# Aedelon/MASt3R-SLAM

Measured on AMD Instinct MI355X. Metric: keyframe-pairs/sec (512x512 two-view infer+match+GN), higher is better.
Workload: dtype fp16

## Files before the change

### include/m3slam_model.h

```cpp
#ifndef M3SLAM_MODEL_H
#define M3SLAM_MODEL_H

#include <stdint.h>

#ifdef __cplusplus
extern "C" {
#endif

enum { M3_DT_BF16 = 0, M3_DT_F16 = 1, M3_DT_F16_PVBF16 = 2 };

enum {
    M3_EPI_BF16 = 0,
    M3_EPI_BF16_GELU = 1,
    M3_EPI_F32 = 2,
    M3_EPI_F32_ACCUM = 3,
    M3_EPI_BF16_RELU = 4,
    M3_EPI_BF16_ADD = 5,
    M3_EPI_BF16_ROPE = 6,
    M3_EPI_INPUT_RELU = 0x100
};

typedef struct m3_gemm_desc {
    const void *A, *W, *W1;
    const float *bias, *bias1;
// ... 29 lines not shown
                             int dtype, void *stream);

int m3_dpt_tail_grouped2_dt(const void *X, const void *Wc0, const void *Wc1, const float *bias0, const float *bias1,
                            const void *W40, const void *W41, const float *b40, const float *b41, float *pts,
                            float *conf, const void *zero16, int B, int H, int Wd, int upsample, int dtype,
                            void *stream);

int m3_conv3x3_up_direct_grouped2_dt(const void *X, const void *W0, const void *W1, const float *bias0,
                                     const float *bias1, void *Y, const void *zero16, int B, int H, int Wd, int Cin,
                                     int upsample, int dtype, void *stream);

int m3_conv3x3_direct_grouped2_dt(const void *X, const void *W0, const void *W1, const float *bias0, const float *bias1,
                                  void *Y, const void *R, const void *zero16, int B, int H, int Wd, int Cin, int Cout,
                                  int epilogue, int dtype, void *stream);

int m3_attention_dt(const void *Q, const void *K, const void *V, void *O, int q_row_stride,
                    int kv_row_stride, int o_row_stride, int64_t q_batch_stride,
                    int64_t kv_batch_stride, int64_t o_batch_stride, int nbatch, int heads,
                    int Tq, int Tk, int kv_batch_shift, float scale, int dtype, void *stream);

int m3_attention_prescaled_dt(const void *Q, const void *K, const void *V, void *O, int q_row_stride,
                              int kv_row_stride, int o_row_stride, int64_t q_batch_stride,
                              int64_t kv_batch_stride, int64_t o_batch_stride, int nbatch, int heads,
                              int Tq, int Tk, int kv_batch_shift, int dtype, void *stream);

int m3_rope2d_dt(void *X, const int32_t *pos_yx, const float *cos_sin, int row_stride, int tokens,
                 int heads, int tokens_per_image, int dtype, void *stream);

int m3_layernorm_dt(const float *x, const float *gamma, const float *beta, void *y, int M, int C,
                    float eps, int dtype, void *stream);
// ... 32 lines not shown
```

### mast3r-slam_amd/csrc/conv_tail.hip

```cpp
#include "gemm_common.h"

using namespace m3gemm;

namespace {

constexpr int kThreads = 512;
constexpr int TH = 16, TW = 32;
constexpr int HH = TH + 2, HW = TW + 2;
constexpr int kHaloPix = HH * HW;
constexpr int kHaloBytes = kHaloPix * 128;
constexpr int kWStage = 128 * 128;
constexpr int PH = 11, PW = 19;
constexpr int kPatchBytes = (PH * PW * 128 + 1023) / 1024 * 1024;
constexpr int kLdsBytes = kHaloBytes + 2 * kWStage + kPatchBytes;

struct TailArgs {
    const bf16_t *X;
    const bf16_t *Wc;
    const float *bias;
    const bf16_t *W4;
    const float *b4;
    float *pts, *conf;
    bf16_t *Y;
    const bf16_t *R;
    int cout, relu_in;
    const bf16_t *zero16;
    int B, H, W, IH, IW;
    const bf16_t *Wc2, *W42;
    const float *bias2, *b42;
};

enum { EP_PLAIN = 0 , EP_TAIL = 1 , EP_RELU = 2 ,
       EP_ADD = 3  };

template <int DT, bool UPS, int CIN, int EP>
__global__ void __launch_bounds__(kThreads, 2)
k_conv_tail(const TailArgs ain) {
    constexpr bool TAIL = EP == EP_TAIL;
    static_assert(CIN % 64 == 0 && (TAIL ? CIN == 128 : true), "64-channel steps; the fused tail is the 128-channel head.2");
    constexpr int NQ = CIN / 64;
    TailArgs a = ain;
    if (blockIdx.y == 1) {
        a.Wc = ain.Wc2; a.W4 = ain.W42; a.bias = ain.bias2; a.b4 = ain.b42;
        a.X = ain.X + (size_t)ain.B * ain.IH * ain.IW * CIN;
        if (TAIL) {
            a.pts = ain.pts + (size_t)ain.B * ain.H * ain.W * 3;
            a.conf = ain.conf + (size_t)ain.B * ain.H * ain.W;
        } else {
            a.Y = ain.Y + (size_t)ain.B * ain.H * ain.W * ain.cout;
            if (EP == EP_ADD) a.R = ain.R + (size_t)ain.B * ain.H * ain.W * ain.cout;
        }
    }
    if (!TAIL) {
        const int z = blockIdx.z;
        a.Wc += (size_t)z * 128 * 9 * CIN;
        if (a.bias) a.bias += z * 128;
        a.Y += z * 128;
        if (EP == EP_ADD) a.R += z * 128;
    }
    extern __shared__ __attribute__((aligned(16))) unsigned char lds[];
    unsigned char *halo = lds, *wst = lds + kHaloBytes, *patch = lds + kHaloBytes + 2 * kWStage;
    const int tid = threadIdx.x, lane = tid & 63, wave = tid >> 6;
    const int wp = wave >> 1, wc = wave & 1;
    const int tiles_x = (a.W + TW - 1) / TW, tiles_y = a.H / TH;
    const int nwg = tiles_x * tiles_y * a.B;
    const int bid = xcd_remap(blockIdx.x, nwg);
    const int b = bid / (tiles_x * tiles_y), trem = bid - b * tiles_x * tiles_y;
    const int ty = trem / tiles_x, tx = trem - ty * tiles_x;
    const int oy0 = ty * TH, ox0 = tx * TW;
    const bf16_t *img = a.X + (size_t)b * a.IH * a.IW * CIN;

    auto stage_w = [&](int tap, int half, int buf) {
        unsigned char *base = wst + buf * kWStage;
#pragma unroll
        for (int i = 0; i < 2; ++i) {
            const int slot = i * kThreads + tid;
            const int row = slot >> 3, cp = slot & 7;
            const int c = half * 8 + (cp ^ ((row >> 1) & 7));
            glds16(a.Wc + ((size_t)row * 9 + tap) * CIN + c * 8, base + i * (kThreads * 16) + wave * 1024);
// ... 47 lines not shown
                q11.q = *reinterpret_cast<const uint4 *>(p + ((y1 - py0) * PW + (x1 - px0)) * 128);
#pragma unroll
                for (int k = 0; k < 4; ++k) {
                    const float tl = lo16<DT>(q00.w[k]) * (1.f - wx) + lo16<DT>(q01.w[k]) * wx;
                    const float bl = lo16<DT>(q10.w[k]) * (1.f - wx) + lo16<DT>(q11.w[k]) * wx;
                    const float th = hi16<DT>(q00.w[k]) * (1.f - wx) + hi16<DT>(q01.w[k]) * wx;
                    const float bh = hi16<DT>(q10.w[k]) * (1.f - wx) + hi16<DT>(q11.w[k]) * wx;
                    r.w[k] = pack16<DT>(tl * (1.f - wy) + bl * wy, th * (1.f - wy) + bh * wy);
                }
                o = r.q;
            }
            *reinterpret_cast<uint4 *>(halo + (size_t)slot * 16) = o;
        }
    };

    f32x4 acc[8][4];
#pragma unroll
    for (int i = 0; i < 8; ++i)
#pragma unroll
        for (int j = 0; j < 4; ++j) acc[i][j] = f32x4{0.f, 0.f, 0.f, 0.f};
    const int frow = lane & 15, fch = lane >> 4;
    int w_off[4];
#pragma unroll
    for (int j = 0; j < 4; ++j) {
        const int r = wc * 64 + j * 16 + frow;
        w_off[j] = r * 128 + ((fch ^ ((r >> 1) & 7)) << 4);
    }

    const int group = wave >> 2;
    bf16x8 af[8], wf[4];
    const int pix_of_row = (int)((0x3D9F2A40E6C851B7ULL >> (4 * frow)) & 15);
    auto col_offset = [&](int hx) { return hx * 128 + ((fch ^ ((hx >> 1) & 7)) << 4); };
    auto read_frags = [&](int g, int tap, int ks) {
        const int ky = tap / 3, kx = tap - ky * 3;
        const unsigned char *wsrc = wst + (g & 1) * kWStage;
        const int flip = ks << 6;
        const int c0 = col_offset(pix_of_row + kx) ^ flip;
        const int c1 = col_offset(16 + pix_of_row + kx) ^ flip;
        const unsigned char *rowp = halo + (wp * 4 + ky) * (HW * 128);
#pragma unroll
        for (int j = 0; j < 4; ++j) wf[j] = *reinterpret_cast<const bf16x8 *>(wsrc + (w_off[j] ^ flip));
#pragma unroll
        for (int i = 0; i < 8; ++i)
            af[i] = *reinterpret_cast<const bf16x8 *>(rowp + (i >> 1) * (HW * 128) + ((i & 1) ? c1 : c0));
        if (!TAIL && a.relu_in) {
#pragma unroll
            for (int i = 0; i < 8; ++i) af[i] = relu_frag(af[i]);
        }
    };
    auto mfma_all = [&]() {
        __builtin_amdgcn_s_setprio(1);
#pragma unroll
        for (int i = 0; i < 8; ++i)
#pragma unroll
            for (int j = 0; j < 4; ++j) acc[i][j] = mfma16<DT>(wf[j], af[i], acc[i][j]);
        __builtin_amdgcn_s_setprio(0);
    };
    auto phase_end = [&]() {
        __builtin_amdgcn_sched_barrier(0);
        __builtin_amdgcn_s_barrier();
        __builtin_amdgcn_sched_barrier(0);
    };
    auto phase_end_wait = [&]() {
        __builtin_amdgcn_sched_barrier(0);
        asm volatile("s_waitcnt vmcnt(0)" ::: "memory");
        __builtin_amdgcn_s_barrier();
        __builtin_amdgcn_sched_barrier(0);
    };
    auto prefetch_w = [&](int g) { if (g + 1 < 9 * NQ) stage_w((g + 1) % 9, (g + 1) / 9, (g + 1) & 1); };
    auto run_half = [&](int half) {
        if (group == 0) {
#pragma unroll 1
            for (int tap = 0; tap < 9; ++tap) {
                const int g = half * 9 + tap;
                read_frags(g, tap, 0);
                prefetch_w(g);
                asm volatile("s_waitcnt lgkmcnt(0)" ::: "memory");
                phase_end();
                mfma_all();
                phase_end();
                read_frags(g, tap, 1);
                asm volatile("s_waitcnt lgkmcnt(0)" ::: "memory");
                phase_end();
                mfma_all();
                phase_end_wait();
            }
            phase_end();
        } else {
#pragma unroll 1
            for (int tap = 0; tap < 9; ++tap) {
                const int g = half * 9 + tap;
                if (tap > 0) mfma_all();
                phase_end();
                read_frags(g, tap, 0);
                prefetch_w(g);
                asm volatile("s_waitcnt lgkmcnt(0)" ::: "memory");
                phase_end();
                mfma_all();
                phase_end();
                read_frags(g, tap, 1);
                asm volatile("s_waitcnt lgkmcnt(0)" ::: "memory");
                phase_end_wait();
            }
            mfma_all();
            phase_end();
        }
    };

    stage_w(0, 0, 0);
    if (UPS) stage_patch(0); else stage_halo_direct(0);
    asm volatile("s_waitcnt vmcnt(0)" ::: "memory");
    lds_barrier();
#pragma unroll 1
    for (int q = 0; q < NQ; ++q) {
        if (UPS) {
            blend_halo();
            lds_barrier();
            if (q + 1 < NQ) stage_patch(q + 1);
        } else if (q > 0) {
            stage_halo_direct(q);
            asm volatile("s_waitcnt vmcnt(0)" ::: "memory");
            lds_barrier();
        }
        run_half(q);
    }

    if constexpr (EP == EP_ADD) {
        const int r = lane & 15, gq = lane >> 4;
        constexpr int RS = 272;
        unsigned char *wl = halo + wave * (32 * RS);
        float4 bj[4];
#pragma unroll
        for (int j = 0; j < 4; ++j)
            bj[j] = a.bias ? *reinterpret_cast<const float4 *>(a.bias + wc * 64 + j * 16 + gq * 4) : make_float4(0.f, 0.f, 0.f, 0.f);
        auto pix = [&](int pass, int rl, int &oy, int &ox) {
            const int i = pass * 2 + (rl >> 4);
            oy = oy0 + wp * 4 + (i >> 1);
            ox = ox0 + (i & 1) * 16 + (int)((0x3D9F2A40E6C851B7ULL >> (4 * (rl & 15))) & 15);
        };
        uint4 q[2][4];
        auto load_resid = [&](int pass, uint4 (&dst)[4]) {
#pragma unroll
            for (int it = 0; it < 4; ++it) {
                const int c = it * 64 + lane, rl = c >> 3, ch = c & 7;
                int oy, ox;
                pix(pass, rl, oy, ox);
                ox = ox < a.W ? ox : a.W - 1;
                dst[it] = *reinterpret_cast<const uint4 *>(a.R + (((size_t)b * a.H + oy) * a.W + ox) * a.cout + wc * 64 + ch * 8);
            }
        };
        load_resid(0, q[0]);
#pragma unroll
        for (int pass = 0; pass < 4; ++pass) {
            if (pass + 1 < 4) load_resid(pass + 1, q[(pass + 1) & 1]);
#pragma unroll
            for (int ii = 0; ii < 2; ++ii)
#pragma unroll
                for (int j = 0; j < 4; ++j) {
                    const f32x4 v = acc[pass * 2 + ii][j];
                    *reinterpret_cast<float4 *>(wl + (ii * 16 + r) * RS + ((j * 4 + gq) << 4)) =
                        make_float4(v[0] + bj[j].x, v[1] + bj[j].y, v[2] + bj[j].z, v[3] + bj[j].w);
                }
            asm volatile("s_waitcnt lgkmcnt(0)" ::: "memory");
#pragma unroll
            for (int it = 0; it < 4; ++it) {
                const int c = it * 64 + lane, rl = c >> 3, ch = c & 7;
                const float4 f0 = *reinterpret_cast<const float4 *>(wl + rl * RS + ch * 32);
                const float4 f1 = *reinterpret_cast<const float4 *>(wl + rl * RS + ch * 32 + 16);
                const uint4 u = q[pass & 1][it];
                uint4 o;
                o.x = pack16<DT>(f0.x + lo16<DT>(u.x), f0.y + hi16<DT>(u.x));
                o.y = pack16<DT>(f0.z + lo16<DT>(u.y), f0.w + hi16<DT>(u.y));
                o.z = pack16<DT>(f1.x + lo16<DT>(u.z), f1.y + hi16<DT>(u.z));
                o.w = pack16<DT>(f1.z + lo16<DT>(u.w), f1.w + hi16<DT>(u.w));
                int oy, ox;
                pix(pass, rl, oy, ox);
                if (ox < a.W)
                    *reinterpret_cast<uint4 *>(a.Y + (((size_t)b * a.H + oy) * a.W + ox) * a.cout + wc * 64 + ch * 8) = o;
            }
            asm volatile("" ::: "memory");
        }
    } else if constexpr (!TAIL) {
        const int r = lane & 15, gq = lane >> 4;
        unsigned char *wl = halo + wave * 8192;
        float4 bj[4];
#pragma unroll
        for (int j = 0; j < 4; ++j)
            bj[j] = a.bias ? *reinterpret_cast<const float4 *>(a.bias + wc * 64 + j * 16 + gq * 4) : make_float4(0.f, 0.f, 0.f, 0.f);
#pragma unroll
        for (int pass = 0; pass < 2; ++pass) {
#pragma unroll
            for (int ii = 0; ii < 4; ++ii)
#pragma unroll
                for (int j = 0; j < 4; ++j) {
                    f32x4 v = acc[pass * 4 + ii][j];
                    v[0] += bj[j].x; v[1] += bj[j].y; v[2] += bj[j].z; v[3] += bj[j].w;
                    if (EP == EP_RELU) {
#pragma unroll
                        for (int e = 0; e < 4; ++e) v[e] = v[e] > 0.f ? v[e] : 0.f;
                    }
                    uint2 pk;
                    pk.x = pack16<DT>(v[0], v[1]); pk.y = pack16<DT>(v[2], v[3]);
                    *reinterpret_cast<uint2 *>(wl + (ii * 16 + r) * 128 + (((j * 2 + (gq >> 1)) ^ ((r >> 1) & 7)) << 4) + (((gq ^ r) & 1) << 3)) = pk;
                }
            asm volatile("s_waitcnt lgkmcnt(0)" ::: "memory");
#pragma unroll
            for (int it = 0; it < 8; ++it) {
                const int c = it * 64 + lane, rl = c >> 3, ch = c & 7;
                uint4 v = *reinterpret_cast<const uint4 *>(wl + rl * 128 + ((ch ^ ((rl >> 1) & 7)) << 4));
                if (rl & 1) v = uint4{v.z, v.w, v.x, v.y};
                const int i = pass * 4 + (rl >> 4);
                const int oy = oy0 + wp * 4 + (i >> 1);
                const int ox = ox0 + (i & 1) * 16 + (int)((0x3D9F2A40E6C851B7ULL >> (4 * (rl & 15))) & 15);
                if (ox < a.W)
                    *reinterpret_cast<uint4 *>(a.Y + (((size_t)b * a.H + oy) * a.W + ox) * a.cout + wc * 64 + ch * 8) = v;
            }
            asm volatile("" ::: "memory");
        }
    } else {
        const int r = lane & 15, gq = lane >> 4;
        float part[8][4];
    #pragma unroll
        for (int i = 0; i < 8; ++i)
    #pragma unroll
            for (int o = 0; o < 4; ++o) part[i][o] = 0.f;
    #pragma unroll
        for (int j = 0; j < 4; ++j) {
            const int n = wc * 64 + j * 16 + gq * 4;
            const float4 bq = a.bias ? *reinterpret_cast<const float4 *>(a.bias + n) : make_float4(0.f, 0.f, 0.f, 0.f);
// ... 36 lines not shown
            if (ox < a.W) {
                const float x = p0.x + p1.x + a.b4[0], y = p0.y + p1.y + a.b4[1];
                const float z = p0.z + p1.z + a.b4[2], c = p0.w + p1.w + a.b4[3];
                const float d = sqrtf(x * x + y * y + z * z);
                const float sc = expm1f(d) / fmaxf(d, 1e-8f);
                const size_t m = ((size_t)b * a.H + oy) * a.W + ox;
                a.pts[3 * m + 0] = x * sc; a.pts[3 * m + 1] = y * sc; a.pts[3 * m + 2] = z * sc;
                a.conf[m] = 1.0f + expf(c);
            }
        }
    }
}

}

extern "C" {

static int dpt_tail_launch(const void *X, const void *Wc, const float *bias, const void *W4, const float *b4,
                           const void *Wc2, const float *bias2, const void *W42, const float *b42, float *pts,
                           float *conf, void *Y, const void *R, const void *zero16, int B, int H, int W, int cin, int cout,
                           int ep, int relu_in, int upsample, int dtype, void *stream) {
    const int groups = Wc2 ? 2 : 1;
    const bool tail = ep == EP_TAIL;
    M3_REQUIRE(X && Wc && zero16 && B > 0 && H > 0 && W > 0 && H % 16 == 0 && W % 16 == 0);
    M3_REQUIRE(tail ? (W4 && b4 && pts && conf && cin == 128 && !Y)
                    : (Y && (cin == 128 || cin == 256) && (cout == 128 || cout == 256) && (ep == EP_PLAIN || ep == EP_RELU || ep == EP_ADD)));
    M3_REQUIRE((ep == EP_ADD) == (R != nullptr) && (!upsample || ep == EP_PLAIN || tail));
    M3_REQUIRE(groups == 1 || ((!tail || (W42 && b42)) && (bias == nullptr) == (bias2 == nullptr)));
    M3_REQUIRE((dtype == DT_BF16 || dtype == DT_F16) && (!upsample || (H % 2 == 0 && W % 2 == 0)));
    M3_REQUIRE((int64_t)groups * B * H * W < (1ll << 31));
    M3_REQUIRE(reinterpret_cast<uintptr_t>(X) % 16 == 0 && reinterpret_cast<uintptr_t>(Wc) % 16 == 0 &&
               reinterpret_cast<uintptr_t>(Y) % 16 == 0 && reinterpret_cast<uintptr_t>(R) % 16 == 0);
    TailArgs a;
    a.Wc2 = (const bf16_t *)Wc2; a.W42 = (const bf16_t *)W42; a.bias2 = bias2; a.b42 = b42;
    a.X = (const bf16_t *)X; a.Wc = (const bf16_t *)Wc; a.bias = bias; a.W4 = (const bf16_t *)W4; a.b4 = b4;
    a.pts = pts; a.conf = conf; a.Y = (bf16_t *)Y; a.R = (const bf16_t *)R; a.cout = tail ? 128 : cout; a.relu_in = relu_in;
    a.zero16 = (const bf16_t *)zero16; a.B = B; a.H = H; a.W = W;
    a.IH = upsample ? H / 2 : H; a.IW = upsample ? W / 2 : W;
    const dim3 grid((unsigned)((H / TH) * ((W + TW - 1) / TW) * B), groups, tail ? 1 : cout / 128), blk(kThreads);
    hipStream_t st = (hipStream_t)stream;
#define M3_TAIL(DTV, UP, CI, EPV)                                                                                \
    do {                                                                                                         \
        static M3AttrOnce once;                                                                                  \
        int dev__;                                                                                               \
        if (m3_attr_need(once, &dev__)) {                                                                        \
            M3_CHECK_HIP(hipFuncSetAttribute(reinterpret_cast<const void *>(&k_conv_tail<DTV, UP, CI, EPV>),     \
                                             hipFuncAttributeMaxDynamicSharedMemorySize, kLdsBytes), "m3_dpt_tail/attr"); \
            m3_attr_done(once, dev__);                                                                           \
        }                                                                                                        \
        hipLaunchKernelGGL((k_conv_tail<DTV, UP, CI, EPV>), grid, blk, kLdsBytes, st, a);                        \
    } while (0)
#define M3_TAIL_DT(UP, CI, EPV) do { if (dtype == DT_F16) M3_TAIL(DT_F16, UP, CI, EPV); else M3_TAIL(DT_BF16, UP, CI, EPV); } while (0)
    if (tail) { if (upsample) M3_TAIL_DT(true, 128, EP_TAIL); else M3_TAIL_DT(false, 128, EP_TAIL); }
    else if (ep == EP_PLAIN && cin == 128) { if (upsample) M3_TAIL_DT(true, 128, EP_PLAIN); else M3_TAIL_DT(false, 128, EP_PLAIN); }
    else if (ep == EP_PLAIN) { if (upsample) M3_TAIL_DT(true, 256, EP_PLAIN); else M3_TAIL_DT(false, 256, EP_PLAIN); }
    else if (ep == EP_RELU) { if (cin == 128) M3_TAIL_DT(false, 128, EP_RELU); else M3_TAIL_DT(false, 256, EP_RELU); }
    else { if (cin == 128) M3_TAIL_DT(false, 128, EP_ADD); else M3_TAIL_DT(false, 256, EP_ADD); }
#undef M3_TAIL_DT
#undef M3_TAIL
    M3_CHECK_LAUNCH("m3_dpt_tail");
    return M3_OK;
}

int m3_dpt_tail_grouped2_dt(const void *X, const void *Wc0, const void *Wc1, const float *bias0, const float *bias1,
                            const void *W40, const void *W41, const float *b40, const float *b41, float *pts,
                            float *conf, const void *zero16, int B, int H, int W, int upsample, int dtype, void *stream) {
    M3_REQUIRE(pts && conf && (Wc1 == nullptr) == (W41 == nullptr));
    if (!Wc1) bias1 = b41 = nullptr;
    return dpt_tail_launch(X, Wc0, bias0, W40, b40, Wc1, bias1, W41, b41, pts, conf, nullptr, nullptr, zero16, B, H, W, 128, 128,
                           EP_TAIL, 0, upsample, dtype, stream);
}

int m3_conv3x3_up_direct_grouped2_dt(const void *X, const void *Wc0, const void *Wc1, const float *bias0, const float *bias1,
                                     void *Y, const void *zero16, int B, int H, int W, int Cin, int upsample, int dtype,
                                     void *stream) {
    M3_REQUIRE(Y != nullptr);
    return dpt_tail_launch(X, Wc0, bias0, nullptr, nullptr, Wc1, Wc1 ? bias1 : nullptr, nullptr, nullptr, nullptr, nullptr, Y,
                           nullptr, zero16, B, H, W, Cin, 128, EP_PLAIN, 0, upsample, dtype, stream);
}

int m3_conv3x3_direct_grouped2_dt(const void *X, const void *W0, const void *W1, const float *bias0, const float *bias1,
                                  void *Y, const void *R, const void *zero16, int B, int H, int W, int Cin, int Cout,
                                  int epilogue, int dtype, void *stream) {
    const int relu_in = (epilogue & 0x100) ? 1 : 0;
    const int e = epilogue & 0xff;
    M3_REQUIRE(Y != nullptr && (e == M3_EPI_BF16 || e == M3_EPI_BF16_RELU || e == M3_EPI_BF16_ADD));
    const int ep = e == M3_EPI_BF16 ? EP_PLAIN : (e == M3_EPI_BF16_RELU ? EP_RELU : EP_ADD);
    return dpt_tail_launch(X, W0, bias0, nullptr, nullptr, W1, bias1, nullptr, nullptr, nullptr, nullptr, Y, R, zero16, B, H, W,
                           Cin, Cout, ep, relu_in, 0, dtype, stream);
}

}
```

### mast3r-slam_amd/csrc/gemm.hip

```cpp
#include <atomic>
#include "gemm_common.h"
#include <cmath>
#include <stdlib.h>

using namespace m3gemm;

namespace {

constexpr int BM = 128, BN = 128;
constexpr int kThreads = 256;

#ifndef M3_GEMM64_STAGES
#define M3_GEMM64_STAGES 2
#endif
constexpr int k_gemm_stages(int T) { return T == 64 ? M3_GEMM64_STAGES : 2; }

template <int MODE , int EPI, int T, int DT, bool SLICED = false>
__global__ void __launch_bounds__(kThreads)
k_gemm(const GemmArgs gin) {
    constexpr int BM = T, BN = T;
    constexpr int NT = T / 32;
    constexpr int kStageBytes = (BM + BN) * BK * 2;
    constexpr int STAGES = k_gemm_stages(T);
    static_assert(4 * (NT == 4 ? 9216 : 4608) + BM * 8 + kRopeTableRows * 128 <= STAGES * kStageBytes, "row table + RoPE table behind the scratch");
// ... 446 lines not shown
        a.rope_pmax = (d->rope_max_pos > 0 && d->rope_max_pos <= kRopeTableRows) ? d->rope_max_pos : 0;
    }
    a.C16 = d->c16; a.stats_out = d->stats_out; a.stats_gstride = d->stats_gstride;
    a.R_lo = d->r_lo; a.C_lo = d->c_lo;
    a.ln_stats = d->ln_stats; a.ln_colsum = d->ln_colsum; a.ln_colsum2 = d->ln_colsum1; a.ln_slots = d->ln_slots;
    a.ln_eps = d->ln_eps; a.ln_gstride = d->ln_gstride;
    if (d->ln_stats) {
        const int top = ln_top_width(d->K);
        a.ln_tops = d->K / top;
        a.ln_gsz = d->ln_slots / a.ln_tops;
    }
    a.stats_w = d->stats_out ? ln_store_width(d->M, d->N, groups) : 0;
    return launch_dense(a, epi, (hipStream_t)stream);
}

int64_t m3_conv3x3_splitk_bytes(int B, int H, int Wd, int Cin, int Cout, int stride) {
    if (B <= 0 || H <= 0 || Wd <= 0 || Cin <= 0 || Cout <= 0 || (stride != 1 && stride != 2)) return 0;
    const int OH = (H + 2 - 3) / stride + 1, OW = (Wd + 2 - 3) / stride + 1;
    const int S = pick_splits(OH * OW, Cout, 9 * Cin);
    return S > 1 ? (int64_t)S * B * OH * OW * Cout * 4 : 0;
}

int m3_conv3x3_grouped2_dt(const void *X, const void *W0, const void *W1, const float *bias0, const float *bias1,
                           void *Y, const void *R, const void *zero16, int B, int H, int Wd, int Cin, int Cout,
                           int stride, int epilogue, void *splitk_ws, int64_t splitk_ws_bytes, int dtype, void *stream) {
    const int relu_in = (epilogue & 0x100) ? 1 : 0;
    epilogue &= 0xff;
    M3_REQUIRE(X && W0 && Y && zero16 && B > 0 && H > 0 && Wd > 0 && Cin > 0 && Cout > 0 && dt_ok(dtype));
    M3_REQUIRE(Cin % BK == 0 && Cout % 4 == 0 && (stride == 1 || stride == 2) && epilogue != EPI_BF16_ROPE);
    M3_REQUIRE(!((epilogue == EPI_F32_ACCUM || epilogue == EPI_BF16_ADD) && !R));
// ... 39 lines not shown
```

### mast3r-slam_amd/mast3r_slam/ops.py

```python
from __future__ import annotations

import os

import ctypes as C

import torch
from torch.utils.weak import WeakTensorKeyDictionary

from . import _ffi

EPI_BF16, EPI_BF16_GELU, EPI_F32, EPI_F32_ACCUM, EPI_BF16_RELU, EPI_BF16_ADD, EPI_BF16_ROPE = range(7)
EPI_INPUT_RELU = 0x100
_F32_EPIS = (EPI_F32, EPI_F32_ACCUM)

_zero16 = {}

H16 = (torch.bfloat16, torch.float16)
DT_CODE = {torch.bfloat16: 0, torch.float16: 1}
DT_F16_PVBF16 = 2


def _pv_code(dt: int, pv_bf16: bool) -> int:
    if not pv_bf16:
        return dt
# ... 96 lines not shown

def conv3x3_ex(x, w, bias=None, epi: int = EPI_BF16, stride: int = 1, resid=None, out=None, relu_input: bool = False, direct=None,
             w1=None, bias1=None):
    x = _ffi.check(x, H16, "x")
    lead = _lead(x, w1, "B,H,W,Cin")
    g = len(lead) + 1
    b, h, wd, cin = x.shape[-4:]
    w = _ffi.check(w, H16, "w", (None, 3, 3, cin))
    cout = w.shape[0]
    w1 = _opt(w1, H16, "w1", tuple(w.shape))
    dt = _same16(x, w, w1)
    oh, ow = (h + 2 - 3) // stride + 1, (wd + 2 - 3) // stride + 1
    odt = torch.float32 if epi in _F32_EPIS else x.dtype
    bias, bias1 = _opt(bias, torch.float32, "bias", (cout,)), _opt(bias1, torch.float32, "bias1", (cout,))
    resid = _opt(resid, odt, "resid", lead + (b, oh, ow, cout))
    if out is None and direct is not False and epi in (EPI_BF16, EPI_BF16_RELU, EPI_BF16_ADD) and (direct or conv3x3_direct_ok(x, cout, stride)):
        return _conv3x3_direct(x, w, w1, bias, bias1, epi, resid, relu_input)
    if out is None:
        out = torch.empty(lead + (b, oh, ow, cout), dtype=odt, device=x.device)
    ws_bytes = g * int(_ffi.lib().m3_conv3x3_splitk_bytes(b, h, wd, cin, cout, stride))
    ws = torch.empty(ws_bytes, dtype=torch.uint8, device=x.device) if ws_bytes > 0 else None
    e0 = _prof_begin()
    _ffi.call("m3_conv3x3_grouped2_dt", _ffi.ptr(x), _ffi.ptr(w), _ffi.ptr(w1), _ffi.ptr(bias), _ffi.ptr(bias1), _ffi.ptr(out),
              _ffi.ptr(resid), _ffi.ptr(zero_page(x.device)), b, h, wd, cin, cout, stride,
              epi | (EPI_INPUT_RELU if relu_input else 0), _ffi.ptr(ws), ws_bytes, dt, _ffi.stream_ptr())
    _prof_end(e0, "conv3x3", 2.0 * g * b * oh * ow * cout * 9 * cin,
              g * (2.0 * (b * h * wd * cin + cout * 9 * cin) + out.element_size() * b * oh * ow * cout * (1 if resid is None else 2)),
              f"conv3x3{' x2' if g == 2 else ''} {b}x{h}x{wd} {cin}->{cout} s{stride} epi{epi} splitk_ws={ws_bytes}")
    return out


def _conv3x3_direct(x, w0, w1, b0, b1, epi, resid, relu_input):
    grouped = x.dim() == 5
    b, h, wd, cin = x.shape[-4:]
    cout = w0.shape[0]
    dt = _same16(x, w0, w1)
    out = torch.empty(tuple(x.shape[:-1]) + (cout,), dtype=x.dtype, device=x.device)
    e0 = _prof_begin()
    _ffi.call("m3_conv3x3_direct_grouped2_dt", _ffi.ptr(x), _ffi.ptr(w0), _ffi.ptr(w1), _ffi.ptr(b0), _ffi.ptr(b1), _ffi.ptr(out),
              _ffi.ptr(resid), _ffi.ptr(zero_page(x.device)), b, h, wd, cin, cout, epi | (EPI_INPUT_RELU if relu_input else 0), dt,
              _ffi.stream_ptr())
    g = 2 if grouped else 1
    _prof_end(e0, "conv_direct", 2.0 * g * b * h * wd * cout * 9 * cin,
              g * (2.0 * (b * h * wd * cin + cout * 9 * cin) + 2.0 * b * h * wd * cout * (1 if resid is None else 2)),
              f"conv3x3 direct{' x2' if grouped else ''} {b}x{h}x{wd} {cin}->{cout} epi{epi}")
    return out


def conv3x3(x: torch.Tensor, w: torch.Tensor, bias=None, epi: int = EPI_BF16, stride: int = 1, resid=None, out=None,
            relu_input: bool = False, direct=None):
    return conv3x3_ex(x, w, bias, epi, stride, resid, out, relu_input, direct)


def conv3x3_grouped2(x, w0, w1, b0, b1, epi: int = EPI_BF16, stride: int = 1, resid=None, relu_input: bool = False, direct=None):
    return conv3x3_ex(x, w0, b0, epi, stride, resid, None, relu_input, direct, w1=_ffi.check(w1, H16, "w1"), bias1=b1)


def conv3x3_relu_head4(x: torch.Tensor, w: torch.Tensor, bias, w4: torch.Tensor, b4: torch.Tensor):
    x = _ffi.check(x, H16, "x")
    b, h, wd, cin = x.shape
# ... 16 lines not shown
DIRECT_CONV_MIN_WGS = None


def _direct_conv_min_wgs() -> int:
    return int(DIRECT_CONV_MIN_WGS) if DIRECT_CONV_MIN_WGS is not None else int(_ffi.lib().m3_device_cu_count())


def conv3x3_direct_ok(x, cout: int, stride: int = 1) -> bool:
    g = 2 if x.dim() == 5 else 1
    b, h, w, cin = x.shape[-4:]
    if stride != 1 or cin not in (128, 256) or cout not in (128, 256) or h % 16 or w % 16 or os.environ.get("M3_DIRECT_CONV", "1") == "0":
        return False
    if int(_ffi.lib().m3_conv3x3_splitk_bytes(1, h, w, cin, cout, 1)) > 0:
        return False
    return (h // 16) * ((w + 31) // 32) * b * (cout // 128) * g >= _direct_conv_min_wgs()


def conv3x3_up_direct_ex(x, w, bias, upsample: bool = True, w1=None, bias1=None):
    x = _ffi.check(x, H16, "x")
    lead = _lead(x, w1, "B,h,w,Cin")
    g = len(lead) + 1
    b, ih, iw, cin = x.shape[-4:]
    w, w1 = _ffi.check(w, H16, "w", (128, 3, 3, cin)), _opt(w1, H16, "w1", (128, 3, 3, cin))
    dt = _same16(x, w, w1)
    bias, bias1 = _opt(bias, torch.float32, "bias", (128,)), _opt(bias1, torch.float32, "bias1", (128,))
    h, wd = (2 * ih, 2 * iw) if upsample else (ih, iw)
    out = torch.empty(lead + (b, h, wd, 128), dtype=x.dtype, device=x.device)
    e0 = _prof_begin()
    _ffi.call("m3_conv3x3_up_direct_grouped2_dt", _ffi.ptr(x), _ffi.ptr(w), _ffi.ptr(w1), _ffi.ptr(bias), _ffi.ptr(bias1), _ffi.ptr(out),
              _ffi.ptr(zero_page(x.device)), b, h, wd, cin, 1 if upsample else 0, dt, _ffi.stream_ptr())
# ... 362 lines not shown
```

Measured before the change: 294.8.

## Add 4-row direct conv tiles with sliced accumulation for small-spatial convs

Adds a 4-row tile variant of the direct 3x3 conv kernel that handles convs which previously fell back to split-K GEMM (Cin 192/384/768, and small spatial sizes). The accumulation is split into slices that are summed in registers to match the split-K summation order. A new routing function picks the tile size from the CU count and the split-K heuristic. It also adds a 16-row path for Cin=192. This avoids the split-K workspace and reduction passes, at the cost of more register pressure and lower per-workgroup reuse.

Result: no change. 295.8 (median of 6 runs) (+0.3%).

```diff
diff --git a/include/m3slam_model.h b/include/m3slam_model.h
--- a/include/m3slam_model.h
+++ b/include/m3slam_model.h
@@ -67,6 +67,14 @@
                                   void *Y, const void *R, const void *zero16, int B, int H, int Wd, int Cin, int Cout,
                                   int epilogue, int dtype, void *stream);
 
+int m3_conv3x3_direct_tile_grouped2_dt(const void *X, const void *W0, const void *W1, const float *bias0, const float *bias1,
+                                       void *Y, const void *R, const void *zero16, int B, int H, int Wd, int Cin, int Cout,
+                                       int epilogue, int tile, int dtype, void *stream);
+
+int m3_conv3x3_small_route(int groups, int B, int H, int Wd, int Cin, int Cout, int stride, int epilogue);
+
+int m3_conv3x3_splits(int pix_per_image, int Cout, int K);
+
 int m3_attention_dt(const void *Q, const void *K, const void *V, void *O, int q_row_stride,
                     int kv_row_stride, int o_row_stride, int64_t q_batch_stride,
                     int64_t kv_batch_stride, int64_t o_batch_stride, int nbatch, int heads,
diff --git a/mast3r-slam_amd/csrc/conv_tail.hip b/mast3r-slam_amd/csrc/conv_tail.hip
--- a/mast3r-slam_amd/csrc/conv_tail.hip
+++ b/mast3r-slam_amd/csrc/conv_tail.hip
@@ -5,14 +5,16 @@
 namespace {
 
 constexpr int kThreads = 512;
-constexpr int TH = 16, TW = 32;
-constexpr int HH = TH + 2, HW = TW + 2;
-constexpr int kHaloPix = HH * HW;
-constexpr int kHaloBytes = kHaloPix * 128;
+constexpr int TW = 32, HW = TW + 2;
+constexpr int halo_bytes(int th) { return (th + 2) * HW * 128; }
 constexpr int kWStage = 128 * 128;
 constexpr int PH = 11, PW = 19;
 constexpr int kPatchBytes = (PH * PW * 128 + 1023) / 1024 * 1024;
-constexpr int kLdsBytes = kHaloBytes + 2 * kWStage + kPatchBytes;
+constexpr int kEpiAddBytes = 8 * 32 * 272;
+constexpr int lds_bytes(int th, bool ups, bool add = false) {
+    const int k = halo_bytes(th) + 2 * kWStage + (ups ? kPatchBytes : 0);
+    return add && k < kEpiAddBytes ? kEpiAddBytes : k;
+}
 
 struct TailArgs {
     const bf16_t *X;
@@ -24,6 +26,7 @@
     bf16_t *Y;
     const bf16_t *R;
     int cout, relu_in;
+    int slices;
     const bf16_t *zero16;
     int B, H, W, IH, IW;
     const bf16_t *Wc2, *W42;
@@ -33,11 +36,16 @@
 enum { EP_PLAIN = 0 , EP_TAIL = 1 , EP_RELU = 2 ,
        EP_ADD = 3  };
 
-template <int DT, bool UPS, int CIN, int EP>
+template <int DT, bool UPS, int CIN, int EP, int TH = 16, bool SLICED = false>
 __global__ void __launch_bounds__(kThreads, 2)
 k_conv_tail(const TailArgs ain) {
     constexpr bool TAIL = EP == EP_TAIL;
     static_assert(CIN % 64 == 0 && (TAIL ? CIN == 128 : true), "64-channel steps; the fused tail is the 128-channel head.2");
+    static_assert((TH == 16 && !SLICED) || (TH == 4 && SLICED && !UPS && !TAIL), "16-row tiles, or 4-row tiles with sliced accumulation");
+    constexpr int HH = TH + 2, kHaloPix = HH * HW, kHaloBytes = halo_bytes(TH);
+    constexpr int RPW = TH / 4;
+    constexpr int NI = 2 * RPW;
+    constexpr int TPP = NI < 4 ? NI : 4;
     constexpr int NQ = CIN / 64;
     TailArgs a = ain;
     if (blockIdx.y == 1) {
@@ -62,7 +70,7 @@
     unsigned char *halo = lds, *wst = lds + kHaloBytes, *patch = lds + kHaloBytes + 2 * kWStage;
     const int tid = threadIdx.x, lane = tid & 63, wave = tid >> 6;
     const int wp = wave >> 1, wc = wave & 1;
-    const int tiles_x = (a.W + TW - 1) / TW, tiles_y = a.H / TH;
+    const int tiles_x = (a.W + TW - 1) / TW, tiles_y = (a.H + TH - 1) / TH;
     const int nwg = tiles_x * tiles_y * a.B;
     const int bid = xcd_remap(blockIdx.x, nwg);
     const int b = bid / (tiles_x * tiles_y), trem = bid - b * tiles_x * tiles_y;
@@ -140,11 +148,28 @@
         }
     };
 
-    f32x4 acc[8][4];
-#pragma unroll
-    for (int i = 0; i < 8; ++i)
+    f32x4 acc[NI][4];
+#pragma unroll
+    for (int i = 0; i < NI; ++i)
 #pragma unroll
         for (int j = 0; j < 4; ++j) acc[i][j] = f32x4{0.f, 0.f, 0.f, 0.f};
+    f32x4 tot[SLICED ? NI : 1][SLICED ? 4 : 1];
+    int slice = 0, slice_end = SLICED ? 9 * NQ * 1 / a.slices : 0;
+    auto fold_slice = [&](int gdone) {
+        if constexpr (SLICED) {
+            if (gdone + 1 == slice_end) {
+#pragma unroll
+                for (int i = 0; i < NI; ++i)
+#pragma unroll
+                    for (int j = 0; j < 4; ++j) {
+                        tot[i][j] = slice == 0 ? acc[i][j] : tot[i][j] + acc[i][j];
+                        acc[i][j] = f32x4{0.f, 0.f, 0.f, 0.f};
+                    }
+                ++slice;
+                slice_end = (int)((long long)(9 * NQ) * (slice + 1) / a.slices);
+            }
+        }
+    };
     const int frow = lane & 15, fch = lane >> 4;
     int w_off[4];
 #pragma unroll
@@ -154,30 +179,31 @@
     }
 
     const int group = wave >> 2;
-    bf16x8 af[8], wf[4];
+    constexpr bool WIDE = TH == 16;
+    bf16x8 af[NI], wf[4], af1[WIDE ? 1 : NI], wf1[WIDE ? 1 : 4];
     const int pix_of_row = (int)((0x3D9F2A40E6C851B7ULL >> (4 * frow)) & 15);
     auto col_offset = [&](int hx) { return hx * 128 + ((fch ^ ((hx >> 1) & 7)) << 4); };
-    auto read_frags = [&](int g, int tap, int ks) {
+    auto read_frags = [&](int g, int tap, int ks, auto &af, auto &wf) {
         const int ky = tap / 3, kx = tap - ky * 3;
         const unsigned char *wsrc = wst + (g & 1) * kWStage;
         const int flip = ks << 6;
         const int c0 = col_offset(pix_of_row + kx) ^ flip;
         const int c1 = col_offset(16 + pix_of_row + kx) ^ flip;
-        const unsigned char *rowp = halo + (wp * 4 + ky) * (HW * 128);
+        const unsigned char *rowp = halo + (wp * RPW + ky) * (HW * 128);
 #pragma unroll
         for (int j = 0; j < 4; ++j) wf[j] = *reinterpret_cast<const bf16x8 *>(wsrc + (w_off[j] ^ flip));
 #pragma unroll
-        for (int i = 0; i < 8; ++i)
+        for (int i = 0; i < NI; ++i)
             af[i] = *reinterpret_cast<const bf16x8 *>(rowp + (i >> 1) * (HW * 128) + ((i & 1) ? c1 : c0));
         if (!TAIL && a.relu_in) {
 #pragma unroll
-            for (int i = 0; i < 8; ++i) af[i] = relu_frag(af[i]);
-        }
-    };
-    auto mfma_all = [&]() {
+            for (int i = 0; i < NI; ++i) af[i] = relu_frag(af[i]);
+        }
+    };
+    auto mfma_all = [&](const auto &af, const auto &wf) {
         __builtin_amdgcn_s_setprio(1);
 #pragma unroll
-        for (int i = 0; i < 8; ++i)
+        for (int i = 0; i < NI; ++i)
 #pragma unroll
             for (int j = 0; j < 4; ++j) acc[i][j] = mfma16<DT>(wf[j], af[i], acc[i][j]);
         __builtin_amdgcn_s_setprio(0);
@@ -194,21 +220,21 @@
         __builtin_amdgcn_sched_barrier(0);
     };
     auto prefetch_w = [&](int g) { if (g + 1 < 9 * NQ) stage_w((g + 1) % 9, (g + 1) / 9, (g + 1) & 1); };
-    auto run_half = [&](int half) {
+    auto run_half_small = [&](int half) {
+        auto read_both = [&](int g, int tap) {
+            read_frags(g, tap, 0, af, wf);
+            read_frags(g, tap, 1, af1, wf1);
+            asm volatile("s_waitcnt lgkmcnt(0)" ::: "memory");
+        };
+        auto mfma_both = [&](int gdone) { mfma_all(af, wf); mfma_all(af1, wf1); fold_slice(gdone); };
         if (group == 0) {
 #pragma unroll 1
             for (int tap = 0; tap < 9; ++tap) {
                 const int g = half * 9 + tap;
-                read_frags(g, tap, 0);
                 prefetch_w(g);
-                asm volatile("s_waitcnt lgkmcnt(0)" ::: "memory");
-                phase_end();
-                mfma_all();
-                phase_end();
-                read_frags(g, tap, 1);
-                asm volatile("s_waitcnt lgkmcnt(0)" ::: "memory");
-                phase_end();
-                mfma_all();
+                read_both(g, tap);
+                phase_end();
+                mfma_both(g);
                 phase_end_wait();
             }
             phase_end();
@@ -216,19 +242,54 @@
 #pragma unroll 1
             for (int tap = 0; tap < 9; ++tap) {
                 const int g = half * 9 + tap;
-                if (tap > 0) mfma_all();
-                phase_end();
-                read_frags(g, tap, 0);
+                prefetch_w(g);
+                if (tap > 0) mfma_both(g - 1);
+                phase_end();
+                read_both(g, tap);
+                phase_end_wait();
+            }
+            mfma_both(half * 9 + 8);
+            phase_end();
+        }
+    };
+    auto run_half = [&](int half) {
+        if constexpr (!WIDE) { run_half_small(half); return; }
+        if (group == 0) {
+#pragma unroll 1
+            for (int tap = 0; tap < 9; ++tap) {
+                const int g = half * 9 + tap;
+                read_frags(g, tap, 0, af, wf);
                 prefetch_w(g);
                 asm volatile("s_waitcnt lgkmcnt(0)" ::: "memory");
                 phase_end();
-                mfma_all();
-                phase_end();
-                read_frags(g, tap, 1);
+                mfma_all(af, wf);
+                phase_end();
+                read_frags(g, tap, 1, af, wf);
+                asm volatile("s_waitcnt lgkmcnt(0)" ::: "memory");
+                phase_end();
+                mfma_all(af, wf);
+                fold_slice(g);
+                phase_end_wait();
+            }
+            phase_end();
+        } else {
+#pragma unroll 1
+            for (int tap = 0; tap < 9; ++tap) {
+                const int g = half * 9 + tap;
+                if (tap > 0) { mfma_all(af, wf); fold_slice(g - 1); }
+                phase_end();
+                read_frags(g, tap, 0, af, wf);
+                prefetch_w(g);
+                asm volatile("s_waitcnt lgkmcnt(0)" ::: "memory");
+                phase_end();
+                mfma_all(af, wf);
+                phase_end();
+                read_frags(g, tap, 1, af, wf);
                 asm volatile("s_waitcnt lgkmcnt(0)" ::: "memory");
                 phase_end_wait();
             }
-            mfma_all();
+            mfma_all(af, wf);
+            fold_slice(half * 9 + 8);
             phase_end();
         }
     };
@@ -250,8 +311,15 @@
         }
         run_half(q);
     }
+    if constexpr (SLICED) {
+#pragma unroll
+        for (int i = 0; i < NI; ++i)
+#pragma unroll
+            for (int j = 0; j < 4; ++j) acc[i][j] = tot[i][j];
+    }
 
     if constexpr (EP == EP_ADD) {
+        static_assert(kEpiAddBytes <= lds_bytes(TH, UPS, true), "epilogue scratch");
         const int r = lane & 15, gq = lane >> 4;
         constexpr int RS = 272;
         unsigned char *wl = halo + wave * (32 * RS);
@@ -261,7 +329,7 @@
             bj[j] = a.bias ? *reinterpret_cast<const float4 *>(a.bias + wc * 64 + j * 16 + gq * 4) : make_float4(0.f, 0.f, 0.f, 0.f);
         auto pix = [&](int pass, int rl, int &oy, int &ox) {
             const int i = pass * 2 + (rl >> 4);
-            oy = oy0 + wp * 4 + (i >> 1);
+            oy = oy0 + wp * RPW + (i >> 1);
             ox = ox0 + (i & 1) * 16 + (int)((0x3D9F2A40E6C851B7ULL >> (4 * (rl & 15))) & 15);
         };
         uint4 q[2][4];
@@ -272,13 +340,14 @@
                 int oy, ox;
                 pix(pass, rl, oy, ox);
                 ox = ox < a.W ? ox : a.W - 1;
+                oy = oy < a.H ? oy : a.H - 1;
                 dst[it] = *reinterpret_cast<const uint4 *>(a.R + (((size_t)b * a.H + oy) * a.W + ox) * a.cout + wc * 64 + ch * 8);
             }
         };
         load_resid(0, q[0]);
 #pragma unroll
-        for (int pass = 0; pass < 4; ++pass) {
-            if (pass + 1 < 4) load_resid(pass + 1, q[(pass + 1) & 1]);
+        for (int pass = 0; pass < NI / 2; ++pass) {
+            if (pass + 1 < NI / 2) load_resid(pass + 1, q[(pass + 1) & 1]);
 #pragma unroll
             for (int ii = 0; ii < 2; ++ii)
 #pragma unroll
@@ -301,25 +370,26 @@
                 o.w = pack16<DT>(f1.z + lo16<DT>(u.w), f1.w + hi16<DT>(u.w));
                 int oy, ox;
                 pix(pass, rl, oy, ox);
-                if (ox < a.W)
+                if (ox < a.W && oy < a.H)
                     *reinterpret_cast<uint4 *>(a.Y + (((size_t)b * a.H + oy) * a.W + ox) * a.cout + wc * 64 + ch * 8) = o;
             }
             asm volatile("" ::: "memory");
         }
     } else if constexpr (!TAIL) {
+        static_assert(8 * TPP * 2048 <= kHaloBytes + 2 * kWStage, "epilogue scratch (4-row tile: over the halo into the dead weight stages)");
         const int r = lane & 15, gq = lane >> 4;
-        unsigned char *wl = halo + wave * 8192;
+        unsigned char *wl = halo + wave * (TPP * 2048);
         float4 bj[4];
 #pragma unroll
         for (int j = 0; j < 4; ++j)
             bj[j] = a.bias ? *reinterpret_cast<const float4 *>(a.bias + wc * 64 + j * 16 + gq * 4) : make_float4(0.f, 0.f, 0.f, 0.f);
 #pragma unroll
-        for (int pass = 0; pass < 2; ++pass) {
-#pragma unroll
-            for (int ii = 0; ii < 4; ++ii)
+        for (int pass = 0; pass < NI / TPP; ++pass) {
+#pragma unroll
+            for (int ii = 0; ii < TPP; ++ii)
 #pragma unroll
                 for (int j = 0; j < 4; ++j) {
-                    f32x4 v = acc[pass * 4 + ii][j];
+                    f32x4 v = acc[pass * TPP + ii][j];
                     v[0] += bj[j].x; v[1] += bj[j].y; v[2] += bj[j].z; v[3] += bj[j].w;
                     if (EP == EP_RELU) {
 #pragma unroll
@@ -331,14 +401,14 @@
                 }
             asm volatile("s_waitcnt lgkmcnt(0)" ::: "memory");
 #pragma unroll
-            for (int it = 0; it < 8; ++it) {
+            for (int it = 0; it < 2 * TPP; ++it) {
                 const int c = it * 64 + lane, rl = c >> 3, ch = c & 7;
                 uint4 v = *reinterpret_cast<const uint4 *>(wl + rl * 128 + ((ch ^ ((rl >> 1) & 7)) << 4));
                 if (rl & 1) v = uint4{v.z, v.w, v.x, v.y};
-                const int i = pass * 4 + (rl >> 4);
-                const int oy = oy0 + wp * 4 + (i >> 1);
+                const int i = pass * TPP + (rl >> 4);
+                const int oy = oy0 + wp * RPW + (i >> 1);
                 const int ox = ox0 + (i & 1) * 16 + (int)((0x3D9F2A40E6C851B7ULL >> (4 * (rl & 15))) & 15);
-                if (ox < a.W)
+                if (ox < a.W && oy < a.H)
                     *reinterpret_cast<uint4 *>(a.Y + (((size_t)b * a.H + oy) * a.W + ox) * a.cout + wc * 64 + ch * 8) = v;
             }
             asm volatile("" ::: "memory");
@@ -405,17 +475,25 @@
 
 }
 
+static bool small_tile_has(int cin, int ep) {
+    return ep == EP_PLAIN ? (cin == 192 || cin == 384 || cin == 768) : ((ep == EP_RELU || ep == EP_ADD) && cin == 256);
+}
+static bool wide_tile_has(int cin, int ep) { return cin == 128 || cin == 256 || (cin == 192 && ep == EP_PLAIN); }
+
 extern "C" {
+
+int m3_conv3x3_splits(int pix_per_image, int Cout, int K);
 
 static int dpt_tail_launch(const void *X, const void *Wc, const float *bias, const void *W4, const float *b4,
                            const void *Wc2, const float *bias2, const void *W42, const float *b42, float *pts,
                            float *conf, void *Y, const void *R, const void *zero16, int B, int H, int W, int cin, int cout,
-                           int ep, int relu_in, int upsample, int dtype, void *stream) {
+                           int ep, int relu_in, int upsample, int dtype, void *stream, int th = 16, int slices = 1) {
     const int groups = Wc2 ? 2 : 1;
     const bool tail = ep == EP_TAIL;
-    M3_REQUIRE(X && Wc && zero16 && B > 0 && H > 0 && W > 0 && H % 16 == 0 && W % 16 == 0);
+    M3_REQUIRE(X && Wc && zero16 && B > 0 && H > 0 && W > 0 && ((H % 16 == 0 && W % 16 == 0) || (!tail && !upsample)));
     M3_REQUIRE(tail ? (W4 && b4 && pts && conf && cin == 128 && !Y)
-                    : (Y && (cin == 128 || cin == 256) && (cout == 128 || cout == 256) && (ep == EP_PLAIN || ep == EP_RELU || ep == EP_ADD)));
+                    : (Y && cout > 0 && cout % 128 == 0 && (ep == EP_PLAIN || ep == EP_RELU || ep == EP_ADD)));
+    M3_REQUIRE(th == 16 ? (wide_tile_has(cin, ep) && slices == 1) : (th == 4 && !tail && !upsample && small_tile_has(cin, ep) && slices >= 1));
     M3_REQUIRE((ep == EP_ADD) == (R != nullptr) && (!upsample || ep == EP_PLAIN || tail));
     M3_REQUIRE(groups == 1 || ((!tail || (W42 && b42)) && (bias == nullptr) == (bias2 == nullptr)));
     M3_REQUIRE((dtype == DT_BF16 || dtype == DT_F16) && (!upsample || (H % 2 == 0 && W % 2 == 0)));
@@ -426,29 +504,47 @@
     a.Wc2 = (const bf16_t *)Wc2; a.W42 = (const bf16_t *)W42; a.bias2 = bias2; a.b42 = b42;
     a.X = (const bf16_t *)X; a.Wc = (const bf16_t *)Wc; a.bias = bias; a.W4 = (const bf16_t *)W4; a.b4 = b4;
     a.pts = pts; a.conf = conf; a.Y = (bf16_t *)Y; a.R = (const bf16_t *)R; a.cout = tail ? 128 : cout; a.relu_in = relu_in;
+    a.slices = slices;
     a.zero16 = (const bf16_t *)zero16; a.B = B; a.H = H; a.W = W;
     a.IH = upsample ? H / 2 : H; a.IW = upsample ? W / 2 : W;
-    const dim3 grid((unsigned)((H / TH) * ((W + TW - 1) / TW) * B), groups, tail ? 1 : cout / 128), blk(kThreads);
+    const int64_t nwg = (int64_t)((H + th - 1) / th) * ((W + TW - 1) / TW) * B;
+    M3_REQUIRE(nwg < (1ll << 31) && cout / 128 <= 65535);
+    const dim3 grid((unsigned)nwg, groups, tail ? 1 : cout / 128), blk(kThreads);
     hipStream_t st = (hipStream_t)stream;
-#define M3_TAIL(DTV, UP, CI, EPV)                                                                                \
+#define M3_TAIL_K(UP, ...)                                                                                       \
     do {                                                                                                         \
         static M3AttrOnce once;                                                                                  \
         int dev__;                                                                                               \
+        constexpr int kLds__ = lds_bytes(th__, UP, add__);                                                            \
         if (m3_attr_need(once, &dev__)) {                                                                        \
-            M3_CHECK_HIP(hipFuncSetAttribute(reinterpret_cast<const void *>(&k_conv_tail<DTV, UP, CI, EPV>),     \
-                                             hipFuncAttributeMaxDynamicSharedMemorySize, kLdsBytes), "m3_dpt_tail/attr"); \
+            M3_CHECK_HIP(hipFuncSetAttribute(reinterpret_cast<const void *>(&k_conv_tail<__VA_ARGS__>),          \
+                                             hipFuncAttributeMaxDynamicSharedMemorySize, kLds__), "m3_dpt_tail/attr"); \
             m3_attr_done(once, dev__);                                                                           \
         }                                                                                                        \
-        hipLaunchKernelGGL((k_conv_tail<DTV, UP, CI, EPV>), grid, blk, kLdsBytes, st, a);                        \
+        hipLaunchKernelGGL((k_conv_tail<__VA_ARGS__>), grid, blk, kLds__, st, a);                                \
     } while (0)
+#define M3_TAIL(DTV, UP, CI, EPV) do { constexpr int th__ = 16; constexpr bool add__ = EPV == EP_ADD; M3_TAIL_K(UP, DTV, UP, CI, EPV); } while (0)
+#define M3_SMALL(DTV, CI, EPV) do { constexpr int th__ = 4; constexpr bool add__ = EPV == EP_ADD; M3_TAIL_K(false, DTV, false, CI, EPV, 4, true); } while (0)
 #define M3_TAIL_DT(UP, CI, EPV) do { if (dtype == DT_F16) M3_TAIL(DT_F16, UP, CI, EPV); else M3_TAIL(DT_BF16, UP, CI, EPV); } while (0)
-    if (tail) { if (upsample) M3_TAIL_DT(true, 128, EP_TAIL); else M3_TAIL_DT(false, 128, EP_TAIL); }
+#define M3_SMALL_DT(CI, EPV) do { if (dtype == DT_F16) M3_SMALL(DT_F16, CI, EPV); else M3_SMALL(DT_BF16, CI, EPV); } while (0)
+    if (th < 16) {
+        if (ep == EP_RELU) M3_SMALL_DT(256, EP_RELU);
+        else if (ep == EP_ADD) M3_SMALL_DT(256, EP_ADD);
+        else if (cin == 192) M3_SMALL_DT(192, EP_PLAIN);
+        else if (cin == 384) M3_SMALL_DT(384, EP_PLAIN);
+        else M3_SMALL_DT(768, EP_PLAIN);
+    }
+    else if (tail) { if (upsample) M3_TAIL_DT(true, 128, EP_TAIL); else M3_TAIL_DT(false, 128, EP_TAIL); }
+    else if (ep == EP_PLAIN && cin == 192) { M3_REQUIRE(!upsample); M3_TAIL_DT(false, 192, EP_PLAIN); }
     else if (ep == EP_PLAIN && cin == 128) { if (upsample) M3_TAIL_DT(true, 128, EP_PLAIN); else M3_TAIL_DT(false, 128, EP_PLAIN); }
     else if (ep == EP_PLAIN) { if (upsample) M3_TAIL_DT(true, 256, EP_PLAIN); else M3_TAIL_DT(false, 256, EP_PLAIN); }
     else if (ep == EP_RELU) { if (cin == 128) M3_TAIL_DT(false, 128, EP_RELU); else M3_TAIL_DT(false, 256, EP_RELU); }
     else { if (cin == 128) M3_TAIL_DT(false, 128, EP_ADD); else M3_TAIL_DT(false, 256, EP_ADD); }
+#undef M3_SMALL_DT
 #undef M3_TAIL_DT
+#undef M3_SMALL
 #undef M3_TAIL
+#undef M3_TAIL_K
     M3_CHECK_LAUNCH("m3_dpt_tail");
     return M3_OK;
 }
@@ -470,15 +566,38 @@
                            nullptr, zero16, B, H, W, Cin, 128, EP_PLAIN, 0, upsample, dtype, stream);
 }
 
+int m3_conv3x3_direct_tile_grouped2_dt(const void *X, const void *W0, const void *W1, const float *bias0, const float *bias1,
+                                       void *Y, const void *R, const void *zero16, int B, int H, int W, int Cin, int Cout,
+                                       int epilogue, int tile, int dtype, void *stream) {
+    const int relu_in = (epilogue & 0x100) ? 1 : 0;
+    const int e = epilogue & 0xff;
+    M3_REQUIRE(Y != nullptr && (e == M3_EPI_BF16 || e == M3_EPI_BF16_RELU || e == M3_EPI_BF16_ADD));
+    M3_REQUIRE(H > 0 && W > 0 && Cin > 0 && Cout > 0 && (tile == 0 || tile == 4 || tile == 16));
+    const int ep = e == M3_EPI_BF16 ? EP_PLAIN : (e == M3_EPI_BF16_RELU ? EP_RELU : EP_ADD);
+    const int S = m3_conv3x3_splits(H * W, Cout, 9 * Cin);
+    if (tile == 0) tile = (S > 1 && small_tile_has(Cin, ep)) || !wide_tile_has(Cin, ep) ? 4 : 16;
+    return dpt_tail_launch(X, W0, bias0, nullptr, nullptr, W1, bias1, nullptr, nullptr, nullptr, nullptr, Y, R, zero16, B, H, W,
+                           Cin, Cout, ep, relu_in, 0, dtype, stream, tile, tile < 16 ? S : 1);
+}
+
 int m3_conv3x3_direct_grouped2_dt(const void *X, const void *W0, const void *W1, const float *bias0, const float *bias1,
                                   void *Y, const void *R, const void *zero16, int B, int H, int W, int Cin, int Cout,
                                   int epilogue, int dtype, void *stream) {
-    const int relu_in = (epilogue & 0x100) ? 1 : 0;
+    return m3_conv3x3_direct_tile_grouped2_dt(X, W0, W1, bias0, bias1, Y, R, zero16, B, H, W, Cin, Cout, epilogue, 0, dtype, stream);
+}
+
+int m3_conv3x3_small_route(int groups, int B, int H, int W, int Cin, int Cout, int stride, int epilogue) {
+    static const bool enabled = [] { const char *e = getenv("M3_CONV_DIRECT_SMALL"); return !(e && atoi(e) == 0); }();
     const int e = epilogue & 0xff;
-    M3_REQUIRE(Y != nullptr && (e == M3_EPI_BF16 || e == M3_EPI_BF16_RELU || e == M3_EPI_BF16_ADD));
+    if (!enabled || stride != 1 || B <= 0 || H <= 0 || W <= 0 || Cin <= 0 || Cout <= 0 || Cout % 128 != 0) return 0;
+    if (e != M3_EPI_BF16 && e != M3_EPI_BF16_RELU && e != M3_EPI_BF16_ADD) return 0;
     const int ep = e == M3_EPI_BF16 ? EP_PLAIN : (e == M3_EPI_BF16_RELU ? EP_RELU : EP_ADD);
-    return dpt_tail_launch(X, W0, bias0, nullptr, nullptr, W1, bias1, nullptr, nullptr, nullptr, nullptr, Y, R, zero16, B, H, W,
-                           Cin, Cout, ep, relu_in, 0, dtype, stream);
-}
-
-}
+    const int g = groups > 1 ? 2 : 1, cus = m3_device_cu_count();
+    const int S = m3_conv3x3_splits(H * W, Cout, 9 * Cin);
+    const int64_t per_tile_col = (int64_t)((W + TW - 1) / TW) * B * (Cout / 128) * g;
+    if (S == 1 && wide_tile_has(Cin, ep) && (Cin != 128 && Cin != 256) && per_tile_col * ((H + 15) / 16) >= cus) return 16;
+    if (S > 1 && small_tile_has(Cin, ep) && per_tile_col * ((H + 3) / 4) >= cus) return 4;
+    return 0;
+}
+
+}
diff --git a/mast3r-slam_amd/csrc/gemm.hip b/mast3r-slam_amd/csrc/gemm.hip
--- a/mast3r-slam_amd/csrc/gemm.hip
+++ b/mast3r-slam_amd/csrc/gemm.hip
@@ -484,6 +484,8 @@
     return launch_dense(a, epi, (hipStream_t)stream);
 }
 
+int m3_conv3x3_splits(int pix_per_image, int Cout, int K) { return pix_per_image > 0 && Cout > 0 && K > 0 ? pick_splits(pix_per_image, Cout, K) : 1; }
+
 int64_t m3_conv3x3_splitk_bytes(int B, int H, int Wd, int Cin, int Cout, int stride) {
     if (B <= 0 || H <= 0 || Wd <= 0 || Cin <= 0 || Cout <= 0 || (stride != 1 && stride != 2)) return 0;
     const int OH = (H + 2 - 3) / stride + 1, OW = (Wd + 2 - 3) / stride + 1;
diff --git a/mast3r-slam_amd/mast3r_slam/ops.py b/mast3r-slam_amd/mast3r_slam/ops.py
--- a/mast3r-slam_amd/mast3r_slam/ops.py
+++ b/mast3r-slam_amd/mast3r_slam/ops.py
@@ -134,8 +134,11 @@
     odt = torch.float32 if epi in _F32_EPIS else x.dtype
     bias, bias1 = _opt(bias, torch.float32, "bias", (cout,)), _opt(bias1, torch.float32, "bias1", (cout,))
     resid = _opt(resid, odt, "resid", lead + (b, oh, ow, cout))
-    if out is None and direct is not False and epi in (EPI_BF16, EPI_BF16_RELU, EPI_BF16_ADD) and (direct or conv3x3_direct_ok(x, cout, stride)):
-        return _conv3x3_direct(x, w, w1, bias, bias1, epi, resid, relu_input)
+    if out is None and direct is not False and epi in (EPI_BF16, EPI_BF16_RELU, EPI_BF16_ADD):
+        tile = 0 if direct is True else int(direct) if direct else 16 if conv3x3_direct_ok(x, cout, stride) else \
+            conv3x3_small_route(x, cout, stride, epi) or None
+        if tile is not None:
+            return _conv3x3_direct(x, w, w1, bias, bias1, epi, resid, relu_input, tile)
     if out is None:
         out = torch.empty(lead + (b, oh, ow, cout), dtype=odt, device=x.device)
     ws_bytes = g * int(_ffi.lib().m3_conv3x3_splitk_bytes(b, h, wd, cin, cout, stride))
@@ -150,20 +153,20 @@
     return out
 
 
-def _conv3x3_direct(x, w0, w1, b0, b1, epi, resid, relu_input):
+def _conv3x3_direct(x, w0, w1, b0, b1, epi, resid, relu_input, tile=0):
     grouped = x.dim() == 5
     b, h, wd, cin = x.shape[-4:]
     cout = w0.shape[0]
     dt = _same16(x, w0, w1)
     out = torch.empty(tuple(x.shape[:-1]) + (cout,), dtype=x.dtype, device=x.device)
     e0 = _prof_begin()
-    _ffi.call("m3_conv3x3_direct_grouped2_dt", _ffi.ptr(x), _ffi.ptr(w0), _ffi.ptr(w1), _ffi.ptr(b0), _ffi.ptr(b1), _ffi.ptr(out),
-              _ffi.ptr(resid), _ffi.ptr(zero_page(x.device)), b, h, wd, cin, cout, epi | (EPI_INPUT_RELU if relu_input else 0), dt,
+    _ffi.call("m3_conv3x3_direct_tile_grouped2_dt", _ffi.ptr(x), _ffi.ptr(w0), _ffi.ptr(w1), _ffi.ptr(b0), _ffi.ptr(b1), _ffi.ptr(out),
+              _ffi.ptr(resid), _ffi.ptr(zero_page(x.device)), b, h, wd, cin, cout, epi | (EPI_INPUT_RELU if relu_input else 0), tile, dt,
               _ffi.stream_ptr())
     g = 2 if grouped else 1
     _prof_end(e0, "conv_direct", 2.0 * g * b * h * wd * cout * 9 * cin,
               g * (2.0 * (b * h * wd * cin + cout * 9 * cin) + 2.0 * b * h * wd * cout * (1 if resid is None else 2)),
-              f"conv3x3 direct{' x2' if grouped else ''} {b}x{h}x{wd} {cin}->{cout} epi{epi}")
+              f"conv3x3 direct{' x2' if grouped else ''} {b}x{h}x{wd} {cin}->{cout} epi{epi} tile{tile}")
     return out
 
 
@@ -210,6 +213,11 @@
     if int(_ffi.lib().m3_conv3x3_splitk_bytes(1, h, w, cin, cout, 1)) > 0:
         return False
     return (h // 16) * ((w + 31) // 32) * b * (cout // 128) * g >= _direct_conv_min_wgs()
+
+
+def conv3x3_small_route(x, cout: int, stride: int = 1, epi: int = EPI_BF16) -> int:
+    b, h, w, cin = x.shape[-4:]
+    return int(_ffi.lib().m3_conv3x3_small_route(2 if x.dim() == 5 else 1, b, h, w, cin, cout, stride, epi))
 
 
 def conv3x3_up_direct_ex(x, w, bias, upsample: bool = True, w1=None, bias1=None):
```
